# kursawe/OpticalFlow

Hardware: AMD Instinct MI355X
Metric: frame-pairs/sec (higher is better)
Workload: dtype f64; 1 GPU; 1024x1024x256 synthetic translating texture (seed 1), speed_alpha=1, remodelling_alpha=1e4, rtol=1e-06, all 255 pairs solved to the stopping rule; frames_per_gpu=256, pairs_in_flight=255, levels=9, coarse_stencils=float8, vcycle_vectors=coarse_float32, w_cycle_level=1, w_cycle_visits=3, warm_start_stride=3, allgather=False, gather_chunks=1, converged=True

## Files before the change

### opticalflow_amd/csrc/vof.hip

```cpp
#include "vof_device.hpp"
#include "vof_sweep0r.hpp"
#include "vof_sweep0p.hpp"
#include "vof_stream0.hpp"
#include "vof_direct.hpp"
#include "vof_boxflow.hpp"
#include "vof_boxsweep.hpp"
#include "vof_blursweep.hpp"
#include "vof_compare.hpp"
#include "vof_liushen.hpp"
#include "vof_preprocess.hpp"
#include "vof_resize.hpp"
#include "../../include/vof.h"

#include <fcntl.h>
#include <unistd.h>

#include <algorithm>
#include <atomic>
#include <cfloat>
#include <chrono>
#include <cmath>
#include <condition_variable>
#include <cstdio>
#include <cstdlib>
// ... 25 lines not shown

struct ProfRec {
    hipEvent_t e0, e1;
    int kid, level, units;
    double bytes;
    double moved;
};

}

struct vof_ctx {
    int device = 0;
    hipStream_t stream = nullptr;
    bool own_stream = false;
    int Ni = 0, Nj = 0, B = 0;
    std::vector<Level> L;
    double *kx = nullptr, *kb = nullptr, *kr = nullptr, *krh = nullptr, *kp = nullptr, *kv = nullptr, *kt = nullptr;
    double* ky = nullptr;
    double* kz = nullptr;
    double* b32 = nullptr;
    bool vfloat = false;
    bool vcoarse32 = false;
    bool l0_handoff = true;
    bool h32 = false;
    const PairParam* pp = nullptr;
    PairParam* pp_buf = nullptr;
    double* warm_x = nullptr;
    size_t warm_cap = 0;
    int* warm_src = nullptr;
    double* partials = nullptr;
    int nblk = 0;
    PairScalars* sc = nullptr;
    int* active = nullptr;
    int* alist = nullptr;
    int alist_n = 0;
    bool use_alist = true;
    double* func3 = nullptr;
    double *W = nullptr, *invT = nullptr;
    int nd = 0;
    int* h_active = nullptr;
    int* h_alist = nullptr;
    PairScalars* h_sc = nullptr;
    double* h_func3 = nullptr;
    char* h_bounce = nullptr;
    hipEvent_t ev_batch[2] = {nullptr, nullptr};
    double* st_movie = nullptr;
    double* st_out[4] = {nullptr, nullptr, nullptr, nullptr};
    double* st_out2[4] = {nullptr, nullptr, nullptr, nullptr};
    hipStream_t copy_stream = nullptr;
    hipEvent_t ev_solved[2] = {nullptr, nullptr}, ev_copied[2] = {nullptr, nullptr}, ev_uploaded[2] = {nullptr, nullptr};
    double* st_movie2 = nullptr;
    double *blur_tmp = nullptr, *blur_w = nullptr, *blur_io = nullptr;
    double* bf_scratch = nullptr;
    double* sw_scratch = nullptr;
    size_t sw_planes = 0;
    bool sw_by_budget = false;
    char* sw_aux = nullptr;
    size_t sw_aux_bytes = 0;
    char* pre_buf = nullptr;
    size_t pre_bytes = 0;
    bool bf_lds_set = false;
    bool bl_lds_set = false;
    bool ls_lds_set = false;
    double* tex_tab = nullptr;
    size_t tex_cap = 0;
    double* gm_V = nullptr;
    GmresState* gm_state = nullptr;
    double* gm_partials = nullptr;
    int* gm_cycle = nullptr;
    int gm_m = 0;
    long long gmres_pairs = 0;
    struct Alloc { void* raw; char* user; size_t bytes; const char* name; int line; };
    std::vector<Alloc> allocs;
    int c_bytes_per_point = 0;
    size_t bytes = 0;
    std::string err;
    const double* frames = nullptr;
    int npairs = 0;
    vof_params prm;
    int cfmt = 0;
    bool fused = true;
    bool fold_stored = false;
    bool fuse_revisit = true;
    bool direct_on = false;
    int dir_cap = 0;
    double *dir_T = nullptr, *dir_tabs = nullptr, *dir_W = nullptr, *dir_r = nullptr, *dir_y = nullptr, *dir_x = nullptr, *dir_t = nullptr;
    int *dir_ipiv = nullptr, *dir_info = nullptr;
    double *dir_R = nullptr, *dir_C = nullptr, *dir_D = nullptr;
    int dir_ld = 0;
    long long direct_pairs = 0;
    bool fuse_rr = true;
    bool fuse_b = true;
    int fused_ends = 3;
    long sweep0r_min_blocks = 512;
    int tail_first = -1;
    size_t tail_lds = 0;
    TailArgs tail;
    int tail_key[6] = {-9, -9, -9, -9, -9, -9};
    bool prof = false;
    int prof_kid = -1, prof_level = -1;
    std::vector<ProfRec> recs;
    std::vector<hipEvent_t> free_events;
    long long prof_dropped = 0;
    double prof_ms[VOF_K_COUNT][16];
    long long prof_n[VOF_K_COUNT][16];
    long long prof_units[VOF_K_COUNT][16];
    double prof_bytes[VOF_K_COUNT][16];
    double prof_moved[VOF_K_COUNT][16];
    int cur_units = 0;
    int dbg_sync = 0;
    long long dbg_seq = 0;
    std::string dbg_fault;
    int dbg_fd = -1;
    bool dbg_canary = false;
    bool dbg_alloc_log = false;
    bool dbg_poison = false;
    size_t part_per_pair = 0;
    vof_ctx* lane_parent = nullptr;
    int lane_lo = 0, lane_slots = 0;
    int dir_ok = -1;
    hipStream_t lane_stream[MAX_LANES] = {};
    hipEvent_t lane_ev[MAX_LANES][2] = {};
    hipEvent_t ev_fork = nullptr;
    hipEvent_t group_ev[MAX_LANES * MAX_LANE_GROUPS] = {};
};

static std::string g_create_error;

namespace {

void dbg_sync_check(vof_ctx* c, const char* what, int level) {
    if (!c->dbg_sync) return;
    ++c->dbg_seq;
    char line[256];
    if (c->dbg_fd >= 0) {
        int n = snprintf(line, sizeof line, "in flight: scope #%lld '%s' level %d, %d pairs, grid %dx%d (%d levels)%-40s\n", c->dbg_seq, what, level,
                         c->cur_units, c->Ni, c->Nj, (int)c->L.size(), "");
        if (pwrite(c->dbg_fd, line, (size_t)n, 0) < 0) {  }
    }
    hipError_t e = hipStreamSynchronize(c->stream);
    hipError_t e2 = hipGetLastError();
    if (e == hipSuccess) e = e2;
    if (e != hipSuccess && c->dbg_fault.empty()) {
        snprintf(line, sizeof line, "VOF_DEBUG_SYNC: scope #%lld, kernel class '%s', level %d, %d pairs, image %dx%d: %s", c->dbg_seq, what, level,
                 c->cur_units, c->Ni, c->Nj, hipGetErrorString(e));
        c->dbg_fault = line;
        fprintf(stderr, "%s\n", line);
        fflush(stderr);
    }
}

struct Prof {
    vof_ctx* c;
    bool on;
    int dkid, dlevel;
    ProfRec rec;
    Prof(vof_ctx* c_, int kid, int level, double bytes_per_pair = 0.0, double moved_per_pair = -1.0) : c(c_), on(false), dkid(kid), dlevel(level) {
        if (!c->prof) return;
        if (c->prof_kid >= 0 && kid != c->prof_kid) return;
        if (c->prof_level >= 0 && level != c->prof_level) return;
        if ((int)c->recs.size() >= MAX_PROF_RECS) { c->prof_dropped++; return; }
        if (c->free_events.size() >= 2) {
            rec.e0 = c->free_events.back(); c->free_events.pop_back();
            rec.e1 = c->free_events.back(); c->free_events.pop_back();
        } else {
            if (hipEventCreate(&rec.e0) != hipSuccess || hipEventCreate(&rec.e1) != hipSuccess) return;
// ... 862 lines not shown
    if (post_pending) {
        VT* third = (VT*)lv.x;
        if (third == x || third == tmp) third = (VT*)lv.x2;
        if (third == x || third == tmp) third = (VT*)lv.r;
        sweep2_level_t<VT>(c, l, x, tmp, third, b, np, active);
        x = third;
    } else if (smooth_level_t<VT>(c, l, x, tmp, b, nu1, np, active, pre, io) != x) std::swap(x, tmp);
    if (io.failed) return x;
    const bool rr_fused = l == 0 && io.rr_done;
    if constexpr (std::is_same<VT, double>::value) {
        if (l == 0 && coarse32_ok(c, nu2)) {
            if (!rr_fused) resrestrict_fine_t<double, float>(c, x, b, (float*)nx.b, np, active);
            float* fx = (float*)nx.x;
            float* ft = (float*)nx.x2;
            const int nu2c = c->prm.nu_post_coarse > 0 ? c->prm.nu_post_coarse : c->prm.nu_post;
            const bool can64 = 1 < last && !(c->tail_first == 1 && tail_prepare(c)) && sweep_st_usable(c, 1) && nu2c > 0;
            const int visits = (c->prm.w_cycle_level == 0 && 1 < last) ? (c->prm.w_cycle_visits > 0 ? c->prm.w_cycle_visits : 2) : 1;
            const bool fr = visits > 1 && revisit_fusable(c, 1);
            float* fe = vcycle_t<float>(c, 1, fx, ft, (const float*)nx.b, np, active, io, true, false, can64 && visits == 1, fr);
            for (int v = 1; v < visits; ++v) {
                float* other = (fe == fx) ? ft : fx;
                fe = vcycle_t<float>(c, 1, fe, other, (const float*)nx.b, np, active, io, false, false, can64 && v == visits - 1,
                                     fr && v < visits - 1, fr);
            }
            SmoothArgs<double> post;
            post.reverse = post.allow_swap = post.final_smooth = true;
            post.ecoarse = (const double*)fe;
            post.ec32 = !can64;
            return smooth_level_t<double>(c, 0, x, tmp, b, nu2, np, active, post, io);
        }
    }
    if (resu) {
        const VT* x_old = (from_zero && nu1 == 1) ? nullptr : tmp;
        resrestrict_u_t<VT>(c, l, x, x_old, (VT*)nx.b, np, active);
    } else if (l == 0 && lv.C == nullptr) {
        if (!rr_fused) resrestrict_fine_t<VT>(c, x, b, (VT*)nx.b, np, active);
    } else {
        apply_level_t<VT>(c, l, x, b, (VT*)lv.r, 1, np, active);
        restrict_level_t<VT>(c, l, (const VT*)lv.r, (VT*)nx.b, np, active);
    }
    VT* cx = (VT*)nx.x;
    VT* ct = (VT*)nx.x2;
    const int visits = (c->prm.w_cycle_level == l && l + 1 < last) ? (c->prm.w_cycle_visits > 0 ? c->prm.w_cycle_visits : 2) : 1;
    const bool fr = visits > 1 && revisit_fusable(c, l + 1);
    VT* ec = vcycle_t<VT>(c, l + 1, cx, ct, (const VT*)nx.b, np, active, io, true, false, false, fr);
    for (int v = 1; v < visits; ++v) {
        VT* other = (ec == cx) ? ct : cx;
        ec = vcycle_t<VT>(c, l + 1, ec, other, (const VT*)nx.b, np, active, io, false, true, false,
                          fr && v < visits - 1, fr);
    }
    SmoothArgs<VT> post;
    post.reverse = post.allow_swap = true;
    post.final_smooth = l == 0;
    post.ecoarse = ec;
    post.out64 = emit64 && l == 1 && std::is_same<VT, float>::value && nu2 > 0;
    if (defer_post) {
        prolong_add_level_t<VT>(c, l, x, ec, np, active);
        return x;
    }
    return smooth_level_t<VT>(c, l, x, tmp, b, nu2, np, active, post, io);
}

template <typename VT> int direct_apply_t(vof_ctx* c, VT* z, const VT* r, int np);

void vcycle(vof_ctx* c, double** xslot, const void* b, int np, ActiveSet active, CycleIO& io) {
    if (c->direct_on) {
        VDISPATCH(c, direct_apply_t<VT>(c, (VT*)*xslot, (const VT*)b, np));
        return;
    }
    void* res = nullptr;
    VDISPATCH(c, res = (void*)vcycle_t<VT>(c, 0, (VT*)*xslot, (VT*)c->L[0].x2, (const VT*)b, np, active, io));
    if (res != (void*)*xslot) {
        c->L[0].x2 = (void*)*xslot;
        *xslot = (double*)res;
    }
}

int build_hierarchy(vof_ctx* c, int np) {
    const vof_params& P = c->prm;
    c->cfmt = P.coarse_precision;
    int nl = (int)c->L.size();
    for (int l = 0; l + 1 < nl; ++l) {
        Level &f = c->L[l], &k = c->L[l + 1];
        dim3 g = grid2d(k.ni, k.nj, np);
        if (l == 0) {
            Prof p(c, VOF_K_GALERKIN0, 0);
            CDISPATCH(c, 1, (k_galerkin<double, CT, true><<<g, blk2d, 0, c->stream>>>(
                                 c->frames, frame_stride(c), c->Nj, P.speed_alpha, P.remodelling_alpha, P.reference_quirks,
                                 nullptr, f.ni, f.nj, (CW*)k.C, k.ni, k.nj, c->pp)));
        } else {
            Prof p(c, VOF_K_GALERKIN, l);
            CDISPATCH(c, 1, (k_galerkin<CT, CT, false><<<g, blk2d, 0, c->stream>>>(
                                 nullptr, 0, 0, 0.0, 0.0, 0, (const CW*)f.C, f.ni, f.nj, (CW*)k.C, k.ni, k.nj, nullptr)));
        }
    }
    return 0;
}

}

namespace vof {
__global__ __launch_bounds__(NT) void k_store_fine_stencil(const double* __restrict__ frames, size_t frame_stride,
                                                           int Nj, double alpha, double beta, int quirks, int ni,
                                                           int nj, double* __restrict__ C,
                                                           const PairParam* __restrict__ pp) {
    int q = blockIdx.x * BX + threadIdx.x, p = blockIdx.y * BY + threadIdx.y, pair = blockIdx.z;
    if (p >= ni || q >= nj) return;
    size_t npts = (size_t)ni * nj, idx = (size_t)p * nj + q;
    int fidx = pair;
    if (pp) { alpha = pp[pair].alpha; beta = pp[pair].beta; fidx = pp[pair].frame; }
    PixCoef k = pix_coef(frames + (size_t)fidx * frame_stride, Nj, p, q, quirks);
    const CLay L(ni, nj);
    double* out = C + (size_t)pair * 81 * L.plane + L.idx(p, q);
    (void)idx;
    npts = L.plane;
    for (int oi = -1; oi <= 1; ++oi)
        for (int oj = -1; oj <= 1; ++oj) {
            double blk[9];
            int tp = p + oi, tq = q + oj;
            if (tp < 0 || tp >= ni || tq < 0 || tq >= nj) {
                for (int t = 0; t < 9; ++t) blk[t] = 0.0;
            } else {
                folded_block(k, alpha, beta, p, q, ni, nj, oi, oj, blk);
            }
            for (int t = 0; t < 9; ++t) out[(size_t)(((oi + 1) * 3 + (oj + 1)) * 9 + t) * npts] = blk[t];
        }
}
}

namespace {

int setup_batch(vof_ctx* c, const double* frames_dev, int np) {
    c->frames = frames_dev;
    c->npairs = np;
    c->cur_units = np;
    int nl = (int)c->L.size();
    if (nl == 1) {
        Level& f = c->L[0];
        Prof p(c, VOF_K_GALERKIN0, 0);
        k_store_fine_stencil<<<grid2d(f.ni, f.nj, np), blk2d, 0, c->stream>>>(
            c->frames, frame_stride(c), c->Nj, c->prm.speed_alpha, c->prm.remodelling_alpha,
            c->prm.reference_quirks, f.ni, f.nj, (double*)f.C, c->pp);
        c->cfmt = 0;
    } else {
        build_hierarchy(c, np);
    }
    Level& last = c->L[nl - 1];
    {
        Prof p(c, VOF_K_COARSE_SETUP, nl - 1);
        CDISPATCH(c, nl - 1, (k_coarse_build<CT><<<np, 256, 0, c->stream>>>((const CW*)last.C, last.ni, last.nj, c->W)));
        dbg_sync_check(c, "coarse_build", nl - 1);
        k_coarse_invert<<<np, 1024, 0, c->stream>>>(c->W, c->nd, c->invT);
    }
    HIPCHK(hipGetLastError());
    return 0;
}

inline dim3 rgrid(const vof_ctx* c, int np) { return dim3(c->nblk, np, 1); }
inline dim3 rgrid(const vof_ctx* c, int np, const ActiveSet& a) { return rgrid(c, pair_slots(c, a, np)); }

int post_active_list(vof_ctx* c, int np) {
    if (!c->use_alist) return 0;
    int n = 0;
    for (int k = 0; k < np; ++k) if (c->h_active[k]) c->h_alist[n++] = k;
    c->alist_n = n;
    if (n) HIPCHK(hipMemcpyAsync(c->alist, c->h_alist, (size_t)n * sizeof(int), hipMemcpyHostToDevice, c->stream));
    return 0;
}

int count_active(vof_ctx* c, int np, bool renew_list = true) {
    if (hipMemcpyAsync(c->h_active, c->active, np * sizeof(int), hipMemcpyDeviceToHost, c->stream) != hipSuccess) return -1;
    if (hipStreamSynchronize(c->stream) != hipSuccess) return -1;
    int n = 0;
    for (int k = 0; k < np; ++k) n += c->h_active[k] != 0;
    if (renew_list && post_active_list(c, np)) return -1;
    return n;
// ... 568 lines not shown
    total += b * nd * 2 * nd + b * nd * nd;
    return total * sizeof(double) + words * 4 + (size_t)B * 3 * 256 * sizeof(double) + 4096;
}

int vof_device_memory(int device_id, size_t* free_bytes, size_t* total_bytes) {
    size_t f = 0, t = 0;
    if (hipSetDevice(device_id) != hipSuccess) return -1;
    if (hipMemGetInfo(&f, &t) != hipSuccess) return -2;
    if (free_bytes) *free_bytes = f;
    if (total_bytes) *total_bytes = t;
    return 0;
}

const char* vof_kernel_name(int k) {
    static const char* names[VOF_K_COUNT] = {"rhs", "apply0", "gs0", "gs", "residual", "restrict", "prolong",
                                             "galerkin0", "galerkin", "coarse_setup", "coarse_solve", "vector",
                                             "reduce", "finalize", "functionals", "coarse_tail", "preprocess"};
    return (k >= 0 && k < VOF_K_COUNT) ? names[k] : "?";
}

void vof_destroy(vof_ctx* c) {
    if (!c) return;
    hipSetDevice(c->device);
    if (c->stream) {
        const hipError_t e = hipStreamSynchronize(c->stream);
        if (e != hipSuccess && (c->dbg_sync || c->dbg_canary))
            fprintf(stderr, "vof_destroy: the context's stream ends with an error: %s\n", hipGetErrorString(e));
    }
    if (c->dbg_canary) {
        std::string rep;
        if (dbg_check_canaries(c, &rep) != 0) { fprintf(stderr, "vof_destroy: VOF_DEBUG_CANARY: %s\n", rep.c_str()); fflush(stderr); }
    }
    if (c->dbg_fd >= 0) close(c->dbg_fd);
    prof_collect(c);
    for (auto e : c->free_events) hipEventDestroy(e);
    for (const auto& a : c->allocs) hipFree(a.raw);
    if (c->h_active) hipHostFree(c->h_active);
    if (c->h_alist) hipHostFree(c->h_alist);
    if (c->h_sc) hipHostFree(c->h_sc);
    if (c->h_func3) hipHostFree(c->h_func3);
    if (c->h_bounce) hipHostFree(c->h_bounce);
    for (int i = 0; i < 2; ++i) if (c->ev_batch[i]) hipEventDestroy(c->ev_batch[i]);
    for (int i = 0; i < 2; ++i) {
        if (c->ev_solved[i]) hipEventDestroy(c->ev_solved[i]);
        if (c->ev_copied[i]) hipEventDestroy(c->ev_copied[i]);
        if (c->ev_uploaded[i]) hipEventDestroy(c->ev_uploaded[i]);
    }
    if (c->copy_stream) hipStreamDestroy(c->copy_stream);
    for (int i = 0; i < MAX_LANES; ++i) {
        if (c->lane_stream[i]) hipStreamDestroy(c->lane_stream[i]);
        for (int j = 0; j < 2; ++j) if (c->lane_ev[i][j]) hipEventDestroy(c->lane_ev[i][j]);
    }
    if (c->ev_fork) hipEventDestroy(c->ev_fork);
    for (hipEvent_t e : c->group_ev) if (e) hipEventDestroy(e);
    if (c->own_stream && c->stream) hipStreamDestroy(c->stream);
    delete c;
}

static int create_impl(vof_ctx* c, int device_id, int n_i, int n_j, int B, void* stream) {
    if (n_i < 4 || n_j < 4) { c->err = "image must be at least 4x4 (the mirror boundary rows need N >= 4)"; return -1; }
    if (B < 1) { c->err = "max_pairs_in_flight must be >= 1"; return -1; }
    int ndev = 0;
    HIPCHK(hipGetDeviceCount(&ndev));
    if (device_id < 0 || device_id >= ndev) { c->err = "no such HIP device"; return -1; }
    HIPCHK(hipSetDevice(device_id));
    c->device = device_id;
    c->Ni = n_i; c->Nj = n_j; c->B = B;
    if (stream) { c->stream = (hipStream_t)stream; c->own_stream = false; }
    else { HIPCHK(hipStreamCreate(&c->stream)); c->own_stream = true; }
    memset(c->prof_ms, 0, sizeof c->prof_ms);
    memset(c->prof_n, 0, sizeof c->prof_n);
    memset(c->prof_units, 0, sizeof c->prof_units);
    memset(c->prof_bytes, 0, sizeof c->prof_bytes);
    memset(c->prof_moved, 0, sizeof c->prof_moved);
    vof_default_params(&c->prm, sizeof c->prm);
    if (const char* e = getenv("VOF_DEBUG_SYNC")) c->dbg_sync = atoi(e);
    if (const char* e = getenv("VOF_DEBUG_CANARY")) c->dbg_canary = e[0] != '0';
    if (const char* e = getenv("VOF_DEBUG_ALLOC_LOG")) c->dbg_alloc_log = e[0] != '0';
    if (const char* e = getenv("VOF_DEBUG_POISON")) c->dbg_poison = e[0] != '0';
    if (c->dbg_sync)
        if (const char* e = getenv("VOF_DEBUG_SYNC_FILE")) c->dbg_fd = open(e, O_WRONLY | O_CREAT, 0644);
    if (const char* e = getenv("VOF_FOLD_STORED")) c->fold_stored = e[0] != '0';
    if (const char* e = getenv("VOF_FUSE_REVISIT")) c->fuse_revisit = e[0] != '0';
    if (const char* e = getenv("VOF_L0_HANDOFF")) c->l0_handoff = e[0] != '0';
    if (const char* e = getenv("VOF_SWEEP0R_MIN_BLOCKS")) c->sweep0r_min_blocks = atol(e);
    if (const char* e = getenv("VOF_ACTIVE_LIST")) c->use_alist = e[0] != '0';
    if (const char* e = getenv("VOF_FUSE_B")) c->fuse_b = e[0] != '0';
    if (const char* e = getenv("VOF_FUSE_RR")) c->fuse_rr = e[0] != '0';
    if (const char* e = getenv("VOF_FUSED_ENDS")) { const int v = atoi(e); if (v >= 0 && v <= 3) c->fused_ends = v; }
    Level l0; l0.ni = n_i - 2; l0.nj = n_j - 2; l0.npts = (size_t)l0.ni * l0.nj;
    c->L.push_back(l0);
    while (std::max(c->L.back().ni, c->L.back().nj) > COARSEST_MAX) {
        Level k; k.ni = (c->L.back().ni + 1) / 2; k.nj = (c->L.back().nj + 1) / 2; k.npts = (size_t)k.ni * k.nj;
        c->L.push_back(k);
    }
    int nl = (int)c->L.size();
    if (nl > 16) { c->err = "too many levels"; return -1; }
    size_t len0 = 3 * l0.npts;
    for (double** v : {&c->kx, &c->kb, &c->kr, &c->krh, &c->kp, &c->kv, &c->kt, &c->ky, &c->kz})
        if (int rc = dev_alloc(c, v, (size_t)B * len0)) return rc;
    for (int l = 0; l < nl; ++l) {
        Level& lv = c->L[l];
        auto valloc = [&](void** q) { double* t = nullptr; int rc = dev_alloc(c, &t, (size_t)B * 3 * lv.npts); *q = t; return rc; };
        if (l + 1 < nl && l > 0) if (int rc = valloc(&lv.r)) return rc;
        if (l + 1 < nl) if (int rc = valloc(&lv.x2)) return rc;
        if (l > 0) {
            if (int rc = valloc(&lv.x)) return rc;
            if (int rc = valloc(&lv.b)) return rc;
        }
        if (nl == 1) {
            double* C = nullptr;
            if (int rc = dev_alloc(c, &C, (size_t)B * 81 * CLay(lv.ni, lv.nj).plane)) return rc;
            lv.C = C;
        }
    }
    if (int rc = ensure_stencil_storage(c, vof_params_default_coarse_precision())) return rc;
    c->nd = 3 * (int)c->L.back().npts;
    {
        int first = -1;
        for (int l = 1; l < nl; ++l) {
            const CLay lay(c->L[l].ni, c->L[l].nj);
            if (c->L[l].npts <= (size_t)TAIL_MAX_PTS && lay.sub <= (size_t)TAIL_MAX_SUB) { first = l; break; }
        }
        if (first >= 0) first = std::max(first, nl - TAIL_MAX_LEVELS);
        if (first >= 1 && first < nl - 1) {
            memset(&c->tail, 0, sizeof c->tail);
            int off = 0;
            for (int l = first; l < nl; ++l) {
                TailLevel& t = c->tail.L[l - first];
                const CLay lay(c->L[l].ni, c->L[l].nj);
                t.ni = c->L[l].ni; t.nj = c->L[l].nj; t.hj = lay.hj; t.sub = (int)lay.sub; t.plane = lay.plane;
                t.xo = off; off += 3 * (t.ni + 2) * (t.nj + 2);
                t.bo = off; off += 3 * t.ni * t.nj;
            }
            c->tail.ro = off; off += 3 * (int)c->L[first].npts;
            c->tail.nl = nl - first;
            c->tail.nd = c->nd;
            c->tail.n_ops = 0;
            c->tail_lds = (size_t)off * sizeof(double);
            if (c->tail_lds <= (size_t)150 * 1024) {
                c->tail_first = first;
                const int lds = (int)c->tail_lds;
                HIPCHK(hipFuncSetAttribute((const void*)k_tail_cycle<CoefB16, double>, hipFuncAttributeMaxDynamicSharedMemorySize, lds));
                HIPCHK(hipFuncSetAttribute((const void*)k_tail_cycle<CoefB16, float>, hipFuncAttributeMaxDynamicSharedMemorySize, lds));
                HIPCHK(hipFuncSetAttribute((const void*)k_tail_cycle<CoefF8, double>, hipFuncAttributeMaxDynamicSharedMemorySize, lds));
                HIPCHK(hipFuncSetAttribute((const void*)k_tail_cycle<CoefF8, float>, hipFuncAttributeMaxDynamicSharedMemorySize, lds));
                HIPCHK(hipFuncSetAttribute((const void*)k_tail_cycle<float, double>, hipFuncAttributeMaxDynamicSharedMemorySize, lds));
                HIPCHK(hipFuncSetAttribute((const void*)k_tail_cycle<float, float>, hipFuncAttributeMaxDynamicSharedMemorySize, lds));
                HIPCHK(hipFuncSetAttribute((const void*)k_tail_cycle<double, double>, hipFuncAttributeMaxDynamicSharedMemorySize, lds));
                HIPCHK(hipFuncSetAttribute((const void*)k_tail_cycle<double, float>, hipFuncAttributeMaxDynamicSharedMemorySize, lds));
            }
        }
    }
    if (int rc = dev_alloc(c, &c->W, (size_t)B * c->nd * 2 * c->nd)) return rc;
    if (int rc = dev_alloc(c, &c->invT, (size_t)B * c->nd * c->nd)) return rc;
    {
        const int lds = 18 * s0_row_bytes(8) + 9 * (S0_W / 2 + 2) * 8;
        HIPCHK(hipFuncSetAttribute((const void*)k_sweep0m<2, true, false, 1>, hipFuncAttributeMaxDynamicSharedMemorySize, lds));
        HIPCHK(hipFuncSetAttribute((const void*)k_sweep0m<2, false, false, 1>, hipFuncAttributeMaxDynamicSharedMemorySize, lds));
        HIPCHK(hipFuncSetAttribute((const void*)k_sweep0m<1, true, false, 1>, hipFuncAttributeMaxDynamicSharedMemorySize, lds));
        HIPCHK(hipFuncSetAttribute((const void*)k_sweep0m<1, false, false, 1>, hipFuncAttributeMaxDynamicSharedMemorySize, lds));
    }
    {
        const int lds = GeoR::RING * 3 * GeoR::W * (int)sizeof(double);
        HIPCHK(hipFuncSetAttribute((const void*)k_sweep_st2<CoefB16, double>, hipFuncAttributeMaxDynamicSharedMemorySize, lds));
        HIPCHK(hipFuncSetAttribute((const void*)k_sweep_st2<CoefF8, double>, hipFuncAttributeMaxDynamicSharedMemorySize, lds));
// ... 2399 lines not shown
```

### opticalflow_amd/csrc/vof_device.hpp

```cpp
#pragma once
#include <hip/hip_runtime.h>
#include <stdint.h>
#include <type_traits>

namespace vof {

constexpr int BX = 64;
constexpr int BY = 4;
constexpr int NT = BX * BY;

struct PairScalars {
    double rho, alpha, omega, beta;
    double bnorm2, rnorm2;
    double tol2;
    int iterations;
    int converged;
    int breakdown;
    int halfstep;
};

struct PairParam {
    double alpha, beta;
    int frame;
    int out;
};

struct ActiveSet {
    const int* flags;
    const int* list;
    __device__ __forceinline__ int pair(int slot) const { return list ? list[slot] : slot; }
    __device__ __forceinline__ bool on(int pair) const { return !flags || flags[pair]; }
};

__device__ __forceinline__ int fold(int t, int n) { return t < 0 ? 1 : (t >= n ? n - 2 : t); }

__device__ __forceinline__ double pweight(int f, int c, int nc) {
    int d = f - 2 * c;
    if (d == 0) return 1.0;
    if (d == -1) return 0.5;
    if (d == 1) return (c + 1 < nc) ? 0.5 : 1.0;
    return 0.0;
}

#ifndef CLAY_PAD
#define CLAY_PAD 1088
#endif
struct CLay {
    int hj;
    size_t sub, plane;
    __host__ __device__ CLay(int ni, int nj) : hj((nj + 1) / 2), sub((size_t)((ni + 1) / 2) * ((nj + 1) / 2)), plane(4 * sub + CLAY_PAD) {}
    __host__ __device__ __forceinline__ size_t idx(int p, int q) const {
        return (size_t)(((p & 1) << 1) | (q & 1)) * sub + (size_t)(p >> 1) * hj + (q >> 1);
    }
};

struct CoefB16 {};
struct CoefF8 {};
template <typename CT> struct CoefFmt { typedef CT word_t; static constexpr int PLANES = 81; static constexpr int ND = 72; };
template <> struct CoefFmt<CoefB16> { typedef uint32_t word_t; static constexpr int PLANES = 45; static constexpr int ND = 36; };
template <> struct CoefFmt<CoefF8> { typedef uint32_t word_t; static constexpr int PLANES = 30; static constexpr int ND = 18; };
template <typename CT> struct CoefPacked { static constexpr bool value = std::is_same<CT, CoefB16>::value || std::is_same<CT, CoefF8>::value; };

__device__ __forceinline__ float f8_decode(uint32_t w, int sel) {
    switch (sel & 3) {
        case 0: return __builtin_amdgcn_cvt_f32_fp8((int)w, 0);
        case 1: return __builtin_amdgcn_cvt_f32_fp8((int)w, 1);
        case 2: return __builtin_amdgcn_cvt_f32_fp8((int)w, 2);
        default: return __builtin_amdgcn_cvt_f32_fp8((int)w, 3);
    }
}
__device__ __forceinline__ float f8_unit(uint32_t ew, int r) {
    return __uint_as_float(((ew >> (8 * r)) & 0xFFu) << 23);
}

__device__ __forceinline__ uint32_t bf16_round(float f) {
    uint32_t u = __float_as_uint(f);
#ifdef VOF_EXP_MANT_BITS
    constexpr int DROP = 23 - VOF_EXP_MANT_BITS;
    return ((u + ((1u << (DROP - 1)) - 1u) + ((u >> DROP) & 1u)) >> DROP) << (DROP - 16);
#else
    return (u + 0x7FFFu + ((u >> 16) & 1u)) >> 16;
#endif
}

template <typename CT> struct CoefSet {
    typedef typename CoefFmt<CT>::word_t word_t;
    static constexpr int PLANES = CoefFmt<CT>::PLANES;
    word_t w[PLANES];
    __device__ __forceinline__ void load(const word_t* __restrict__ sp, size_t plane) {
#pragma unroll
        for (int k = 0; k < PLANES; ++k) w[k] = sp[(size_t)k * plane];
    }
    __device__ __forceinline__ void load_u(const word_t* __restrict__ ubase, size_t plane, unsigned idx) {
#pragma unroll
        for (int k = 0; k < PLANES; ++k) w[k] = (ubase + (size_t)k * plane)[idx];
    }
    __device__ __forceinline__ void clear() {
#pragma unroll
        for (int k = 0; k < PLANES; ++k) w[k] = 0;
    }
    __device__ __forceinline__ double get(int i) const {
        if constexpr (std::is_same<CT, CoefB16>::value) {
            const int d = i / 9, e = i - 9 * d;
            if (d == 4) return (double)__uint_as_float(w[36 + e]);
            const int j = (d < 4 ? d : d - 1) * 9 + e;
            const uint32_t v = w[j >> 1];
            return (double)__uint_as_float((j & 1) ? (v & 0xFFFF0000u) : (v << 16));
        } else if constexpr (std::is_same<CT, CoefF8>::value) {
            const int d = i / 9, e = i - 9 * d;
            if (d == 4) return (double)__uint_as_float(w[18 + e]);
            const int j = (d < 4 ? d : d - 1) * 9 + e;
            return (double)(f8_decode(w[j >> 2], j & 3) * f8_unit(w[27 + e / 3], e % 3));
        } else {
            return (double)w[i];
        }
    }
};
template <typename CT>
__device__ __forceinline__ double coef_at(const typename CoefFmt<CT>::word_t* __restrict__ Cp, size_t plane, size_t idx, int i) {
    if constexpr (std::is_same<CT, CoefB16>::value) {
        const int d = i / 9, e = i - 9 * d;
        if (d == 4) return (double)__uint_as_float(Cp[(size_t)(36 + e) * plane + idx]);
        const int j = (d < 4 ? d : d - 1) * 9 + e;
        const uint32_t v = Cp[(size_t)(j >> 1) * plane + idx];
        return (double)__uint_as_float((j & 1) ? (v & 0xFFFF0000u) : (v << 16));
    } else if constexpr (std::is_same<CT, CoefF8>::value) {
        const int d = i / 9, e = i - 9 * d;
        if (d == 4) return (double)__uint_as_float(Cp[(size_t)(18 + e) * plane + idx]);
        const int j = (d < 4 ? d : d - 1) * 9 + e;
        const uint32_t v = Cp[(size_t)(j >> 2) * plane + idx] >> (8 * (j & 3));
        return (double)(__builtin_amdgcn_cvt_f32_fp8((int)v, 0) * f8_unit(Cp[(size_t)(27 + e / 3) * plane + idx], e % 3));
    } else {
        return (double)Cp[(size_t)i * plane + idx];
    }
}

struct PixCoef {
    double P, Dx, Dy, Dxx, Dyy, Dxy;
};
struct PixCoefF {
    float P, Dx, Dy, Dxx, Dyy, Dxy;
    __device__ __forceinline__ PixCoefF() {}
    __device__ __forceinline__ explicit PixCoefF(const PixCoef& k)
        : P((float)k.P), Dx((float)k.Dx), Dy((float)k.Dy), Dxx((float)k.Dxx), Dyy((float)k.Dyy), Dxy((float)k.Dxy) {}
};

__device__ __forceinline__ PixCoef pix_coef(const double* __restrict__ I, int Nj, int p, int q, int quirks) {
    const double* c = I + (size_t)(p + 1) * Nj + (q + 1);
    double i00 = c[0];
    double im0 = c[-Nj], ip0 = c[Nj], i0m = c[-1], i0p = c[1];
    double imm = c[-Nj - 1], imp = c[-Nj + 1], ipm = c[Nj - 1], ipp = c[Nj + 1];
    PixCoef k;
    k.P = i00;
    k.Dx = (ip0 - im0) / 2;
    k.Dy = quirks ? k.Dx : (i0p - i0m) / 2;
    k.Dxx = ip0 + im0 - 2 * i00;
    k.Dyy = i0p + i0m - 2 * i00;
    k.Dxy = (ipp - ipm - imp + imm) / 4;
    return k;
}

template <typename T, typename KT>
__device__ __forceinline__ void add_raw_block(const KT& k, T alpha, T beta, int oi, int oj, T scale, T* blk) {
    const T P = k.P;
    if (oi == 0 && oj == 0) {
        blk[0] += scale * (P * (k.Dxx + -2 * P) - 4 * alpha);
        blk[1] += scale * (P * k.Dxy);
        blk[3] += scale * (P * k.Dxy);
        blk[4] += scale * (P * (k.Dyy + -2 * P) - 4 * alpha);
        blk[6] += scale * k.Dx;
        blk[7] += scale * k.Dy;
        blk[8] += scale * (-1 - 4 * beta);
    } else if (oj == 0) {
        T s = (T)oi;
        blk[0] += scale * (P * (s * k.Dx + P) + alpha);
        blk[1] += scale * (s * P * k.Dy / 2);
        blk[2] += scale * (-s * P / 2);
        blk[3] += scale * (s * P * k.Dy / 2);
        blk[4] += scale * alpha;
        blk[6] += scale * (s * P / 2);
        blk[8] += scale * beta;
    } else if (oi == 0) {
        T s = (T)oj;
        blk[0] += scale * alpha;
        blk[1] += scale * (s * P * k.Dx / 2);
        blk[3] += scale * (s * P * k.Dx / 2);
        blk[4] += scale * (P * (s * k.Dy + P) + alpha);
        blk[5] += scale * (-s * P / 2);
        blk[7] += scale * (s * P / 2);
        blk[8] += scale * beta;
    } else {
        T s = (T)(oi * oj);
        blk[1] += scale * (s * P * P / 4);
        blk[3] += scale * (s * P * P / 4);
    }
}

__host__ __device__ constexpr unsigned raw_block_mask(int oi, int oj) {
    return (oi == 0 && oj == 0) ? 0x1DBu
         : (oj == 0)            ? 0x15Fu
         : (oi == 0)            ? 0x1BBu
                                : 0x00Au;
}

template <typename T, typename KT>
__device__ __forceinline__ void folded_block(const KT& k, T alpha, T beta, int p, int q, int ni, int nj, int oi, int oj, T* blk) {
#pragma unroll
    for (int t = 0; t < 9; ++t) blk[t] = (T)0;
    bool gi = (oi == 1 && p == 0) || (oi == -1 && p == ni - 1);
    bool gj = (oj == 1 && q == 0) || (oj == -1 && q == nj - 1);
    add_raw_block(k, alpha, beta, oi, oj, (T)1, blk);
    if (gi) add_raw_block(k, alpha, beta, -oi, oj, (T)1, blk);
    if (gj) add_raw_block(k, alpha, beta, oi, -oj, (T)1, blk);
    if (gi && gj) add_raw_block(k, alpha, beta, -oi, -oj, (T)2, blk);
}

struct Nbr {
    double u[9], w[9], g[9];
};

template <typename XT>
__device__ __forceinline__ void load_nbr(const XT* __restrict__ x, size_t npts, int ni, int nj, int p, int q,
                                         Nbr& n) {
#pragma unroll
    for (int di = -1; di <= 1; ++di) {
        int tp = p + di;
        bool oi = (tp < 0) || (tp >= ni);
        int fp = fold(tp, ni);
#pragma unroll
        for (int dj = -1; dj <= 1; ++dj) {
            int tq = q + dj;
            bool oj = (tq < 0) || (tq >= nj);
            int fq = fold(tq, nj);
            size_t idx = (size_t)fp * nj + fq;
            double s = (oi && oj) ? 2.0 : 1.0;
            int t = (di + 1) * 3 + (dj + 1);
            n.u[t] = s * (double)x[idx];
            n.w[t] = s * (double)x[npts + idx];
            if (di == 0 || dj == 0) n.g[t] = s * (double)x[2 * npts + idx];
        }
    }
}

__device__ __forceinline__ void offdiag0(const PixCoef& k, double alpha, double beta, const Nbr& n, double& y0,
                                         double& y1, double& y2) {
    const double P = k.P;
    const double hPDx = P * k.Dx / 2, hPDy = P * k.Dy / 2, qPP = P * P / 4, hP = P / 2;
    y0 = (P * (P - k.Dx) + alpha) * n.u[1] + (P * (P + k.Dx) + alpha) * n.u[7] + alpha * (n.u[3] + n.u[5]) +
         hPDx * (n.w[5] - n.w[3]) + hPDy * (n.w[7] - n.w[1]) + qPP * ((n.w[8] - n.w[2]) - (n.w[6] - n.w[0])) +
         hP * (n.g[1] - n.g[7]);
    y1 = (P * (P - k.Dy) + alpha) * n.w[3] + (P * (P + k.Dy) + alpha) * n.w[5] + alpha * (n.w[1] + n.w[7]) +
         hPDy * (n.u[7] - n.u[1]) + hPDx * (n.u[5] - n.u[3]) + qPP * ((n.u[8] - n.u[2]) - (n.u[6] - n.u[0])) +
         hP * (n.g[3] - n.g[5]);
    y2 = beta * (n.g[1] + n.g[7] + n.g[3] + n.g[5]) + hP * (n.u[7] - n.u[1]) + hP * (n.w[5] - n.w[3]);
}

struct Diag0 { double axx, ayy, c, inv; };
struct VDiff0 { double du71, dw71, U4, W4; };
template <bool CORNERS, int ZERO = 0, int DC = 0, int PRE = 0>
__device__ __forceinline__ void gs0_point(const double* im, const Nbr& n, double sUL, double sUR, double sDL, double sDR,
                                          double alpha, double beta, double inv_g, int quirks, double b0, double b1,
                                          double b2, double& u, double& w, double& gm, Diag0* dg = nullptr,
                                          const VDiff0* vd = nullptr) {
#pragma clang fp contract(off)
    const double P = im[4];
    const double Dx = (im[7] - im[1]) * 0.5;
    const double Dy = quirks ? Dx : (im[5] - im[3]) * 0.5;
    const double PP = P * P, PDx = P * Dx, PDy = P * Dy, hP = 0.5 * P;
    const double A1 = PP + alpha, qPP = 0.25 * PP, hPDx = 0.5 * PDx, hPDy = 0.5 * PDy;
    double r0, r1, r2;
    if (ZERO == 1) {
        r0 = b0; r1 = b1; r2 = b2;
    } else if (ZERO == 2) {
        const double du53 = n.u[5] - n.u[3], dw53 = n.w[5] - n.w[3];
        const double y0a = fma(hPDx, dw53, alpha * (n.u[3] + n.u[5]));
        const double y1a = A1 * (n.w[3] + n.w[5]);
        const double y1b = fma(hP, n.g[3] - n.g[5], fma(hPDx, du53, PDy * dw53));
        const double y2 = fma(hP, dw53, beta * (n.g[3] + n.g[5]));
        r0 = b0 - y0a; r1 = b1 - (y1a + y1b); r2 = b2 - y2;
    } else {
        double du71, dw71, W4, U4;
        if (PRE) {
            du71 = vd->du71; dw71 = vd->dw71; U4 = vd->U4; W4 = vd->W4;
        } else {
            du71 = n.u[7] - n.u[1]; dw71 = n.w[7] - n.w[1];
            if (CORNERS) {
// ... 324 lines not shown
            const int q = fq + cc - 1;
            const bool qok = on && q >= 0 && q < nj;
            const unsigned uq = qok ? (unsigned)q : 0u;
#pragma unroll
            for (int a = 0; a < 3; ++a) {
                if (a == 1 && !with_mid) continue;
                const bool ok = qok && xrok[a];
#pragma unroll
                for (int f = 0; f < 3; ++f) {
                    double v = (double)(xn + (size_t)f * npts + xrow[a])[uq];
                    if (HAS_OLD) v -= (double)(xo + (size_t)f * npts + xrow[a])[uq];
                    dl[a][cc][f] = ok ? v : 0.0;
                }
            }
        };
        load_col(1, false); load_col(2, true); load_col(3, false);
        double acc0, acc1, acc2;
        {
            double r10 = 0.0, r11 = 0.0, r12 = 0.0;
            CoefSet<CT> cs;
            coef_load_blocks<CT, 0x1C7u>(cs, c1row, L.plane, ucq, on && fq + 1 < nj);
#pragma unroll
            for (int a = 0; a < 3; a += 2)
#pragma unroll
                for (int b = 0; b < 3; ++b) {
                    const int t0 = (a * 3 + b) * 9;
                    const double xu = dl[a][b + 1][0], xw = dl[a][b + 1][1], xg = dl[a][b + 1][2];
                    r10 -= cs.get(t0 + 0) * xu + cs.get(t0 + 1) * xw + cs.get(t0 + 2) * xg;
                    r11 -= cs.get(t0 + 3) * xu + cs.get(t0 + 4) * xw + cs.get(t0 + 5) * xg;
                    r12 -= cs.get(t0 + 6) * xu + cs.get(t0 + 7) * xw + cs.get(t0 + 8) * xg;
                }
            double l0 = __shfl_up(r10, 1), l1 = __shfl_up(r11, 1), l2 = __shfl_up(r12, 1);
            if (lane == 0) { l0 = carry0; l1 = carry1; l2 = carry2; }
            carry0 = __shfl(r10, BX - 1); carry1 = __shfl(r11, BX - 1); carry2 = __shfl(r12, BX - 1);
            const double wjR = (cq + 1 < ncj) ? 0.5 : 1.0;
            acc0 = 0.5 * l0 + wjR * r10; acc1 = 0.5 * l1 + wjR * r11; acc2 = 0.5 * l2 + wjR * r12;
        }
        RESU_PHASE_FENCE();
        load_col(0, true);
#pragma unroll
        for (int side = 0; side < 2; ++side) {
            const int a = side ? 2 : 0;
            CoefSet<CT> cs;
            coef_load_blocks<CT, 0x028u>(cs, side ? c2rowD : c2rowU, L.plane, ucq, on && (side ? rowD : rowU));
            double s0 = 0.0, s1 = 0.0, s2 = 0.0;
#pragma unroll
            for (int b = 0; b < 3; b += 2) {
                const int t0 = (3 + b) * 9;
                const double xu = dl[a][b][0], xw = dl[a][b][1], xg = dl[a][b][2];
                s0 -= cs.get(t0 + 0) * xu + cs.get(t0 + 1) * xw + cs.get(t0 + 2) * xg;
                s1 -= cs.get(t0 + 3) * xu + cs.get(t0 + 4) * xw + cs.get(t0 + 5) * xg;
                s2 -= cs.get(t0 + 6) * xu + cs.get(t0 + 7) * xw + cs.get(t0 + 8) * xg;
            }
            const double wi = side ? wiD : wiU;
            acc0 += wi * s0; acc1 += wi * s1; acc2 += wi * s2;
        }
        RESU_PHASE_FENCE();
        {
            CoefSet<CT> cs;
            coef_load_blocks<CT, 0x1EFu>(cs, c0row, L.plane, ucq, on);
            double r00 = 0.0, r01 = 0.0, r02 = 0.0;
#pragma unroll
            for (int a = 0; a < 3; ++a)
#pragma unroll
                for (int b = 0; b < 3; ++b) {
                    if (a == 1 && b == 1) continue;
                    const int t0 = (a * 3 + b) * 9;
                    const double xu = dl[a][b][0], xw = dl[a][b][1], xg = dl[a][b][2];
                    r00 -= cs.get(t0 + 0) * xu + cs.get(t0 + 1) * xw + cs.get(t0 + 2) * xg;
                    r01 -= cs.get(t0 + 3) * xu + cs.get(t0 + 4) * xw + cs.get(t0 + 5) * xg;
                    r02 -= cs.get(t0 + 6) * xu + cs.get(t0 + 7) * xw + cs.get(t0 + 8) * xg;
                }
            acc0 += r00; acc1 += r01; acc2 += r02;
        }
        if (on) {
            out[cq] = (VT)(0.25 * acc0);
            out[nc + cq] = (VT)(0.25 * acc1);
            out[2 * nc + cq] = (VT)(0.25 * acc2);
        }
        RESU_PHASE_FENCE();
    }
}

template <typename CTF, typename CTC, bool LEVEL0>
__global__ __launch_bounds__(NT) void k_galerkin(const double* __restrict__ frames, size_t frame_stride, int Nj,
                                                 double alpha, double beta, int quirks,
                                                 const typename CoefFmt<CTF>::word_t* __restrict__ Cf, int nfi, int nfj,
                                                 typename CoefFmt<CTC>::word_t* __restrict__ Cc, int nci, int ncj,
                                                 const PairParam* __restrict__ pp) {
    int cq = blockIdx.x * BX + threadIdx.x, cp = blockIdx.y * BY + threadIdx.y;
    int pair = blockIdx.z;
    if (cp >= nci || cq >= ncj) return;
    int fidx = pair;
    if (LEVEL0 && pp) { alpha = pp[pair].alpha; beta = pp[pair].beta; fidx = pp[pair].frame; }
    const CLay Lf(nfi, nfj), Lc(nci, ncj);
    const size_t nf = Lf.plane, nc = Lc.plane;
    typedef typename std::conditional<std::is_same<CTC, double>::value, double, float>::type AT;
    AT acc[9][9];
#pragma unroll
    for (int d = 0; d < 9; ++d)
#pragma unroll
        for (int t = 0; t < 9; ++t) acc[d][t] = (AT)0;
    const bool interior = cp >= 1 && cp + 1 < nci && 2 * cp + 1 <= nfi - 2 && cq >= 1 && cq + 1 < ncj && 2 * cq + 1 <= nfj - 2;
    auto accumulate = [&](auto interior_tag) {
        constexpr bool IN = decltype(interior_tag)::value;
#pragma unroll
        for (int fi = -1; fi <= 1; ++fi) {
            const int fp = 2 * cp + fi;
            if (!IN && (fp < 0 || fp >= nfi)) continue;
            const double wfi = IN ? (fi == 0 ? 1.0 : 0.5) : pweight(fp, cp, nci);
#pragma unroll
            for (int fj = -1; fj <= 1; ++fj) {
                const int fq = 2 * cq + fj;
                if (!IN && (fq < 0 || fq >= nfj)) continue;
                const double wf = wfi * (IN ? (fj == 0 ? 1.0 : 0.5) : pweight(fq, cq, ncj));
                PixCoef k;
                PixCoefF kf;
                CoefSet<CTF> fs;
                if (LEVEL0) { k = pix_coef(frames + (size_t)fidx * frame_stride, Nj, fp, fq, quirks); kf = PixCoefF(k); }
                else fs.load(Cf + (size_t)pair * CoefFmt<CTF>::PLANES * nf + Lf.idx(fp, fq), nf);
#pragma unroll
                for (int oi = -1; oi <= 1; ++oi) {
                    const int gp = fp + oi;
                    if (!IN && (gp < 0 || gp >= nfi)) continue;
#pragma unroll
                    for (int oj = -1; oj <= 1; ++oj) {
                        const int gq = fq + oj;
                        if (!IN && (gq < 0 || gq >= nfj)) continue;
                        AT blk[9];
                        if (LEVEL0) {
                            if (IN) {
#pragma unroll
                                for (int t = 0; t < 9; ++t) blk[t] = (AT)0;
                                if constexpr (std::is_same<AT, float>::value) add_raw_block(kf, (float)alpha, (float)beta, oi, oj, 1.0f, blk);
                                else add_raw_block(k, alpha, beta, oi, oj, 1.0, blk);
                            } else {
                                if constexpr (std::is_same<AT, float>::value) folded_block(kf, (float)alpha, (float)beta, fp, fq, nfi, nfj, oi, oj, blk);
                                else folded_block(k, alpha, beta, fp, fq, nfi, nfj, oi, oj, blk);
                            }
                        } else {
#pragma unroll
                            for (int t = 0; t < 9; ++t) blk[t] = (AT)fs.get(((oi + 1) * 3 + (oj + 1)) * 9 + t);
                        }
#pragma unroll
                        for (int a = -1; a <= 1; ++a) {
                            const int ti = fi + oi - 2 * a;
                            if (ti < -1 || ti > 1) continue;
                            const int Dp = cp + a;
                            if (!IN && (Dp < 0 || Dp >= nci)) continue;
                            const double wgi = IN ? (ti == 0 ? 1.0 : 0.5) : pweight(gp, Dp, nci);
#pragma unroll
                            for (int b = -1; b <= 1; ++b) {
                                const int tj = fj + oj - 2 * b;
                                if (tj < -1 || tj > 1) continue;
                                const int Dq = cq + b;
                                if (!IN && (Dq < 0 || Dq >= ncj)) continue;
                                const AT w = (AT)(wf * wgi * (IN ? (tj == 0 ? 1.0 : 0.5) : pweight(gq, Dq, ncj)));
#pragma unroll
                                for (int t = 0; t < 9; ++t) {
                                    if (LEVEL0 && !((raw_block_mask(oi, oj) >> t) & 1u)) continue;
                                    acc[(a + 1) * 3 + (b + 1)][t] += w * blk[t];
                                }
                            }
                        }
                    }
                }
            }
        }
    };
    if constexpr (LEVEL0) {
        if (interior) accumulate(std::true_type{}); else accumulate(std::false_type{});
    } else {
        accumulate(std::false_type{});
    }
    typename CoefFmt<CTC>::word_t* out = Cc + (size_t)pair * CoefFmt<CTC>::PLANES * nc + Lc.idx(cp, cq);
    if constexpr (std::is_same<CTC, CoefB16>::value) {
        float diag[9];
#pragma unroll
        for (int t = 0; t < 9; ++t) diag[t] = 0.25f * acc[4][t];
        uint32_t h[72];
#pragma unroll
        for (int d = 0; d < 9; ++d) {
            if (d == 4) continue;
#pragma unroll
            for (int t = 0; t < 9; ++t) {
                const float v = 0.25f * acc[d][t];
                const uint32_t hb = bf16_round(v);
                diag[t] += v - __uint_as_float(hb << 16);
                h[(d < 4 ? d : d - 1) * 9 + t] = hb;
            }
        }
#pragma unroll
        for (int j = 0; j < 36; ++j) out[(size_t)j * nc] = h[2 * j] | (h[2 * j + 1] << 16);
#pragma unroll
        for (int t = 0; t < 9; ++t) out[(size_t)(36 + t) * nc] = __float_as_uint(diag[t]);
    } else if constexpr (std::is_same<CTC, CoefF8>::value) {
        float diag[9], amax[9];
#pragma unroll
        for (int t = 0; t < 9; ++t) { diag[t] = 0.25f * acc[4][t]; amax[t] = 0.f; }
#pragma unroll
        for (int d = 0; d < 9; ++d) {
            if (d == 4) continue;
#pragma unroll
            for (int t = 0; t < 9; ++t) amax[t] = fmaxf(amax[t], fabsf(0.25f * acc[d][t]));
        }
        uint32_t ew[3] = {0u, 0u, 0u};
        float unit[9], inv[9];
#pragma unroll
        for (int t = 0; t < 9; ++t) {
            int eb = (int)((__float_as_uint(amax[t]) >> 23) & 0xFFu) - 6;
            eb = eb < 1 ? 1 : (eb > 253 ? 253 : eb);
            ew[t / 3] |= (uint32_t)eb << (8 * (t % 3));
            unit[t] = __uint_as_float((uint32_t)eb << 23);
            inv[t] = __uint_as_float((uint32_t)(254 - eb) << 23);
        }
        float sv[72];
#pragma unroll
        for (int d = 0; d < 9; ++d) {
            if (d == 4) continue;
#pragma unroll
            for (int t = 0; t < 9; ++t) sv[(d < 4 ? d : d - 1) * 9 + t] = 0.25f * acc[d][t] * inv[t];
        }
#pragma unroll
        for (int k = 0; k < 18; ++k) {
            int w = 0;
            w = __builtin_amdgcn_cvt_pk_fp8_f32(sv[4 * k], sv[4 * k + 1], w, false);
            w = __builtin_amdgcn_cvt_pk_fp8_f32(sv[4 * k + 2], sv[4 * k + 3], w, true);
#pragma unroll
            for (int u = 0; u < 4; ++u) {
                const int j = 4 * k + u, t = j % 9;
                diag[t] += (sv[j] - f8_decode((uint32_t)w, u)) * unit[t];
            }
            out[(size_t)k * nc] = (uint32_t)w;
        }
#pragma unroll
        for (int t = 0; t < 9; ++t) out[(size_t)(18 + t) * nc] = __float_as_uint(diag[t]);
#pragma unroll
        for (int r = 0; r < 3; ++r) out[(size_t)(27 + r) * nc] = ew[r];
    } else {
#pragma unroll
        for (int d = 0; d < 9; ++d)
#pragma unroll
            for (int t = 0; t < 9; ++t) out[(size_t)(d * 9 + t) * nc] = (CTC)((AT)0.25 * acc[d][t]);
    }
}

template <typename CT>
__global__ void k_coarse_build(const typename CoefFmt<CT>::word_t* __restrict__ C, int ni, int nj, double* __restrict__ W) {
    int pair = blockIdx.x;
    int npts = ni * nj, nd = 3 * npts;
    double* Wp = W + (size_t)pair * nd * 2 * nd;
    for (int t = threadIdx.x; t < nd * 2 * nd; t += blockDim.x) {
        int row = t / (2 * nd), col = t % (2 * nd);
        Wp[t] = (col == nd + row) ? 1.0 : 0.0;
// ... 2483 lines not shown
```

Measured before the change: 1459 frame-pairs/s.

## Split level-0 Galerkin into interior and border kernels, add closed-form coarse stencil

Level-0 Galerkin coarsening now launches a dedicated interior kernel using the branch-free accumulation path, followed by a compact border-only kernel that maps a linear thread index onto the boundary ring of coarse points. An optional variant (bit 2 of a new env flag, off by default) replaces the triple-nested restriction/prolongation accumulation with compile-time precomputed closed-form coefficients applied to per-pixel image products. The aim is to remove per-thread interior branching and divergence in the coarse operator build. The split adds an extra launch, and the closed-form path may change float rounding order.

```diff
diff --git a/opticalflow_amd/csrc/vof.hip b/opticalflow_amd/csrc/vof.hip
--- a/opticalflow_amd/csrc/vof.hip
+++ b/opticalflow_amd/csrc/vof.hip
@@ -131,6 +131,7 @@
     bool fused = true;
     bool fold_stored = false;
     bool fuse_revisit = true;
+    int galerkin_fast = 1;
     bool direct_on = false;
     int dir_cap = 0;
     double *dir_T = nullptr, *dir_tabs = nullptr, *dir_W = nullptr, *dir_r = nullptr, *dir_y = nullptr, *dir_x = nullptr, *dir_t = nullptr;
@@ -1159,16 +1160,27 @@
     int nl = (int)c->L.size();
     for (int l = 0; l + 1 < nl; ++l) {
         Level &f = c->L[l], &k = c->L[l + 1];
-        dim3 g = grid2d(k.ni, k.nj, np);
+        const dim3 g = grid2d(k.ni, k.nj, np);
         if (l == 0) {
             Prof p(c, VOF_K_GALERKIN0, 0);
-            CDISPATCH(c, 1, (k_galerkin<double, CT, true><<<g, blk2d, 0, c->stream>>>(
+            const GalerkinFrame frame(f.ni, f.nj, k.ni, k.nj);
+            const bool split = frame.any_interior() && (c->galerkin_fast & 1);
+            const dim3 gb = split ? dim3((frame.border_points(k.ni, k.nj) + NT - 1) / NT, 1, np) : g;
+            if (split && (c->galerkin_fast & 2))
+                CDISPATCH(c, 1, (k_galerkin<double, CT, true, true, true><<<g, blk2d, 0, c->stream>>>(
+                                     c->frames, frame_stride(c), c->Nj, P.speed_alpha, P.remodelling_alpha, P.reference_quirks,
+                                     nullptr, f.ni, f.nj, (CW*)k.C, k.ni, k.nj, c->pp, 0)));
+            else if (split)
+                CDISPATCH(c, 1, (k_galerkin<double, CT, true, true><<<g, blk2d, 0, c->stream>>>(
+                                     c->frames, frame_stride(c), c->Nj, P.speed_alpha, P.remodelling_alpha, P.reference_quirks,
+                                     nullptr, f.ni, f.nj, (CW*)k.C, k.ni, k.nj, c->pp, 0)));
+            CDISPATCH(c, 1, (k_galerkin<double, CT, true, false><<<gb, blk2d, 0, c->stream>>>(
                                  c->frames, frame_stride(c), c->Nj, P.speed_alpha, P.remodelling_alpha, P.reference_quirks,
-                                 nullptr, f.ni, f.nj, (CW*)k.C, k.ni, k.nj, c->pp)));
+                                 nullptr, f.ni, f.nj, (CW*)k.C, k.ni, k.nj, c->pp, split ? 1 : 0)));
         } else {
             Prof p(c, VOF_K_GALERKIN, l);
-            CDISPATCH(c, 1, (k_galerkin<CT, CT, false><<<g, blk2d, 0, c->stream>>>(
-                                 nullptr, 0, 0, 0.0, 0.0, 0, (const CW*)f.C, f.ni, f.nj, (CW*)k.C, k.ni, k.nj, nullptr)));
+            CDISPATCH(c, 1, (k_galerkin<CT, CT, false, false><<<g, blk2d, 0, c->stream>>>(
+                                 nullptr, 0, 0, 0.0, 0.0, 0, (const CW*)f.C, f.ni, f.nj, (CW*)k.C, k.ni, k.nj, nullptr, 0)));
         }
     }
     return 0;
@@ -1903,6 +1915,7 @@
         if (const char* e = getenv("VOF_DEBUG_SYNC_FILE")) c->dbg_fd = open(e, O_WRONLY | O_CREAT, 0644);
     if (const char* e = getenv("VOF_FOLD_STORED")) c->fold_stored = e[0] != '0';
     if (const char* e = getenv("VOF_FUSE_REVISIT")) c->fuse_revisit = e[0] != '0';
+    if (const char* e = getenv("VOF_GALERKIN_FAST")) c->galerkin_fast = atoi(e) & 3;
     if (const char* e = getenv("VOF_L0_HANDOFF")) c->l0_handoff = e[0] != '0';
     if (const char* e = getenv("VOF_SWEEP0R_MIN_BLOCKS")) c->sweep0r_min_blocks = atol(e);
     if (const char* e = getenv("VOF_ACTIVE_LIST")) c->use_alist = e[0] != '0';
diff --git a/opticalflow_amd/csrc/vof_device.hpp b/opticalflow_amd/csrc/vof_device.hpp
--- a/opticalflow_amd/csrc/vof_device.hpp
+++ b/opticalflow_amd/csrc/vof_device.hpp
@@ -2,6 +2,7 @@
 #include <hip/hip_runtime.h>
 #include <stdint.h>
 #include <type_traits>
+#include <utility>
 
 namespace vof {
 
@@ -161,7 +162,7 @@
 }
 
 template <typename T, typename KT>
-__device__ __forceinline__ void add_raw_block(const KT& k, T alpha, T beta, int oi, int oj, T scale, T* blk) {
+__host__ __device__ __forceinline__ constexpr void add_raw_block(const KT& k, T alpha, T beta, int oi, int oj, T scale, T* blk) {
     const T P = k.P;
     if (oi == 0 && oj == 0) {
         blk[0] += scale * (P * (k.Dxx + -2 * P) - 4 * alpha);
@@ -202,6 +203,98 @@
          : (oi == 0)            ? 0x1BBu
                                 : 0x00Au;
 }
+
+enum RawField { RF_PP, RF_PDX, RF_PDY, RF_PDXX, RF_PDYY, RF_PDXY, RF_P, RF_DX, RF_DY, RF_IMAGE ,
+                RF_ALPHA = RF_IMAGE, RF_BETA, RF_ONE, RF_ALL };
+__host__ __device__ constexpr double raw_block_coef(int m, int oi, int oj, int t) {
+    if (oi == 0 && oj == 0) {
+        if (t == 0) return m == RF_PDXX ? 1 : m == RF_PP ? -2 : m == RF_ALPHA ? -4 : 0;
+        if (t == 1 || t == 3) return m == RF_PDXY ? 1 : 0;
+        if (t == 4) return m == RF_PDYY ? 1 : m == RF_PP ? -2 : m == RF_ALPHA ? -4 : 0;
+        if (t == 6) return m == RF_DX ? 1 : 0;
+        if (t == 7) return m == RF_DY ? 1 : 0;
+        if (t == 8) return m == RF_ONE ? -1 : m == RF_BETA ? -4 : 0;
+    } else if (oj == 0) {
+        const double s = oi;
+        if (t == 0) return m == RF_PDX ? s : (m == RF_PP || m == RF_ALPHA) ? 1 : 0;
+        if (t == 1 || t == 3) return m == RF_PDY ? s / 2 : 0;
+        if (t == 2) return m == RF_P ? -s / 2 : 0;
+        if (t == 4) return m == RF_ALPHA ? 1 : 0;
+        if (t == 6) return m == RF_P ? s / 2 : 0;
+        if (t == 8) return m == RF_BETA ? 1 : 0;
+    } else if (oi == 0) {
+        const double s = oj;
+        if (t == 0) return m == RF_ALPHA ? 1 : 0;
+        if (t == 1 || t == 3) return m == RF_PDX ? s / 2 : 0;
+        if (t == 4) return m == RF_PDY ? s : (m == RF_PP || m == RF_ALPHA) ? 1 : 0;
+        if (t == 5) return m == RF_P ? -s / 2 : 0;
+        if (t == 7) return m == RF_P ? s / 2 : 0;
+        if (t == 8) return m == RF_BETA ? 1 : 0;
+    } else {
+        if (t == 1 || t == 3) return m == RF_PP ? (double)(oi * oj) / 4 : 0;
+    }
+    return 0;
+}
+template <typename T, typename KT>
+__host__ __device__ __forceinline__ constexpr void raw_fields(const KT& k, T* phi) {
+    const T P = k.P;
+    phi[RF_PP] = P * P; phi[RF_PDX] = P * k.Dx; phi[RF_PDY] = P * k.Dy; phi[RF_PDXX] = P * k.Dxx; phi[RF_PDYY] = P * k.Dyy;
+    phi[RF_PDXY] = P * k.Dxy; phi[RF_P] = P; phi[RF_DX] = k.Dx; phi[RF_DY] = k.Dy;
+}
+__host__ __device__ constexpr bool raw_block_coef_matches(const PixCoef& k, double alpha, double beta) {
+    double phi[RF_ALL] = {};
+    raw_fields(k, phi);
+    phi[RF_ALPHA] = alpha; phi[RF_BETA] = beta; phi[RF_ONE] = 1;
+    for (int oi = -1; oi <= 1; ++oi)
+        for (int oj = -1; oj <= 1; ++oj) {
+            double blk[9] = {};
+            add_raw_block(k, alpha, beta, oi, oj, 1.0, blk);
+            for (int t = 0; t < 9; ++t) {
+                double v = 0;
+                bool any = false;
+                for (int m = 0; m < RF_ALL; ++m) {
+                    const double s = raw_block_coef(m, oi, oj, t);
+                    any = any || s != 0;
+                    v += s * phi[m];
+                }
+                if (v != blk[t]) return false;
+                if (any != (((raw_block_mask(oi, oj) >> t) & 1u) != 0)) return false;
+            }
+        }
+    return true;
+}
+static_assert(raw_block_coef_matches(PixCoef{3, 5, 7, 11, 13, 17}, 19, 23), "raw_block_coef is not add_raw_block");
+static_assert(raw_block_coef_matches(PixCoef{0, 0, 0, 0, 0, 0}, 19, 23), "constant terms of raw_block_coef are not those of add_raw_block");
+static_assert(raw_block_coef_matches(PixCoef{0, 0, 0, 0, 0, 0}, 0, 0), "the 1 part of raw_block_coef is not that of add_raw_block");
+
+struct GalerkinClosedForm {
+    double k[RF_ALL][3][3][9][9];
+    double c[3][9][9];
+};
+__host__ __device__ constexpr double galerkin_w(int d) { return d == 0 ? 1.0 : ((d == 1 || d == -1) ? 0.5 : 0.0); }
+__host__ __device__ constexpr GalerkinClosedForm make_galerkin_closed_form() {
+    GalerkinClosedForm K = {};
+    for (int oi = -1; oi <= 1; ++oi)
+        for (int oj = -1; oj <= 1; ++oj)
+            for (int t = 0; t < 9; ++t)
+                for (int m = 0; m < RF_ALL; ++m) {
+                    const double s = raw_block_coef(m, oi, oj, t);
+                    if (s == 0) continue;
+                    for (int fi = -1; fi <= 1; ++fi)
+                        for (int fj = -1; fj <= 1; ++fj)
+                            for (int a = -1; a <= 1; ++a)
+                                for (int b = -1; b <= 1; ++b) {
+                                    const double w = galerkin_w(fi) * galerkin_w(fj) * galerkin_w(fi + oi - 2 * a) * galerkin_w(fj + oj - 2 * b);
+                                    K.k[m][fi + 1][fj + 1][(a + 1) * 3 + (b + 1)][t] += w * s;
+                                    if (m >= RF_IMAGE) K.c[m - RF_IMAGE][(a + 1) * 3 + (b + 1)][t] += w * s;
+                                }
+                }
+    return K;
+}
+template <typename F, int... I>
+__device__ __forceinline__ void static_for_impl(F&& f, std::integer_sequence<int, I...>) { (f(std::integral_constant<int, I>{}), ...); }
+template <int N, typename F>
+__device__ __forceinline__ void static_for(F&& f) { static_for_impl(f, std::make_integer_sequence<int, N>{}); }
 
 template <typename T, typename KT>
 __device__ __forceinline__ void folded_block(const KT& k, T alpha, T beta, int p, int q, int ni, int nj, int oi, int oj, T* blk) {
@@ -692,15 +785,48 @@
     }
 }
 
-template <typename CTF, typename CTC, bool LEVEL0>
+inline constexpr GalerkinClosedForm kGalerkinClosedForm = make_galerkin_closed_form();
+struct GalerkinFrame {
+    int pi, qi;
+    __host__ __device__ GalerkinFrame(int nfi, int nfj, int nci, int ncj) {
+        const int a = nfi >= 3 ? (nfi - 3) / 2 : 0, b = nfj >= 3 ? (nfj - 3) / 2 : 0;
+        pi = nci - 2 < a ? nci - 2 : a;
+        qi = ncj - 2 < b ? ncj - 2 : b;
+        if (pi < 1 || qi < 1) pi = qi = 0;
+    }
+    __host__ __device__ bool any_interior() const { return pi >= 1; }
+    __host__ __device__ bool interior(int cp, int cq) const { return cp >= 1 && cp <= pi && cq >= 1 && cq <= qi; }
+    __host__ __device__ int border_points(int nci, int ncj) const { return (nci - pi) * ncj + pi * (ncj - qi); }
+    __host__ __device__ void border_point(int t, int nci, int ncj, int& cp, int& cq) const {
+        const int rows = (nci - pi) * ncj;
+        if (t < rows) {
+            const int r = t / ncj;
+            cq = t - r * ncj;
+            cp = r == 0 ? 0 : pi + r;
+        } else {
+            const int cols = ncj - qi, u = t - rows, r = u / cols, c = u - r * cols;
+            cp = 1 + r;
+            cq = c == 0 ? 0 : qi + c;
+        }
+    }
+};
+template <typename CTF, typename CTC, bool LEVEL0, bool FAST, bool CLOSED = false>
 __global__ __launch_bounds__(NT) void k_galerkin(const double* __restrict__ frames, size_t frame_stride, int Nj,
                                                  double alpha, double beta, int quirks,
                                                  const typename CoefFmt<CTF>::word_t* __restrict__ Cf, int nfi, int nfj,
                                                  typename CoefFmt<CTC>::word_t* __restrict__ Cc, int nci, int ncj,
-                                                 const PairParam* __restrict__ pp) {
+                                                 const PairParam* __restrict__ pp, const int border_only) {
+    static_assert((LEVEL0 || !FAST) && (FAST || !CLOSED), "the interior kernel exists for level 0 only, the closed form in it only");
     int cq = blockIdx.x * BX + threadIdx.x, cp = blockIdx.y * BY + threadIdx.y;
     int pair = blockIdx.z;
+    const GalerkinFrame frame(nfi, nfj, nci, ncj);
+    if (!FAST && border_only) {
+        const int t = blockIdx.x * NT + threadIdx.y * BX + threadIdx.x;
+        if (t >= frame.border_points(nci, ncj)) return;
+        frame.border_point(t, nci, ncj, cp, cq);
+    }
     if (cp >= nci || cq >= ncj) return;
+    if (FAST && !frame.interior(cp, cq)) return;
     int fidx = pair;
     if (LEVEL0 && pp) { alpha = pp[pair].alpha; beta = pp[pair].beta; fidx = pp[pair].frame; }
     const CLay Lf(nfi, nfj), Lc(nci, ncj);
@@ -711,7 +837,6 @@
     for (int d = 0; d < 9; ++d)
 #pragma unroll
         for (int t = 0; t < 9; ++t) acc[d][t] = (AT)0;
-    const bool interior = cp >= 1 && cp + 1 < nci && 2 * cp + 1 <= nfi - 2 && cq >= 1 && cq + 1 < ncj && 2 * cq + 1 <= nfj - 2;
     auto accumulate = [&](auto interior_tag) {
         constexpr bool IN = decltype(interior_tag)::value;
 #pragma unroll
@@ -778,8 +903,28 @@
             }
         }
     };
-    if constexpr (LEVEL0) {
-        if (interior) accumulate(std::true_type{}); else accumulate(std::false_type{});
+    auto closed_form = [&](auto) {
+        const AT al = (AT)alpha, be = (AT)beta;
+        static_for<81>([&](auto E) {
+            constexpr int e = decltype(E)::value;
+            constexpr double ka = kGalerkinClosedForm.c[0][e / 9][e % 9], kb = kGalerkinClosedForm.c[1][e / 9][e % 9], k1 = kGalerkinClosedForm.c[2][e / 9][e % 9];
+            if constexpr (ka != 0.0 || kb != 0.0 || k1 != 0.0) acc[e / 9][e % 9] = al * (AT)ka + be * (AT)kb + (AT)k1;
+        });
+        static_for<9>([&](auto F) {
+            constexpr int fi = decltype(F)::value / 3, fj = decltype(F)::value % 3;
+            const PixCoef k = pix_coef(frames + (size_t)fidx * frame_stride, Nj, 2 * cp + fi - 1, 2 * cq + fj - 1, quirks);
+            AT phi[RF_IMAGE];
+            if constexpr (std::is_same<AT, float>::value) raw_fields(PixCoefF(k), phi);
+            else raw_fields(k, phi);
+            static_for<81 * RF_IMAGE>([&](auto X) {
+                constexpr int m = decltype(X)::value % RF_IMAGE, e = decltype(X)::value / RF_IMAGE;
+                constexpr double kv = kGalerkinClosedForm.k[m][decltype(F)::value / 3][decltype(F)::value % 3][e / 9][e % 9];
+                if constexpr (kv != 0.0) acc[e / 9][e % 9] += (AT)kv * phi[m];
+            });
+        });
+    };
+    if constexpr (FAST) {
+        if constexpr (CLOSED) closed_form(0); else accumulate(std::true_type{});
     } else {
         accumulate(std::false_type{});
     }
```

Result: faster. 1484 frame-pairs/s (median of 6 runs) (+1.7%).
